# oscar-youngquist/HCR_Genesis_LR_CL

Hardware: AMD Instinct MI355X
Metric: env-steps/sec, Go2 flat 12-DOF, 4096 envs @1/2/4/8 MI355X (higher is better)
Workload: dtype f32

## Files before the change

### hcr_genesis_lr_cl_amd/build.py

```python
import hashlib
import json
import os
import subprocess
import sys
from concurrent.futures import ThreadPoolExecutor

HERE = os.path.dirname(os.path.abspath(__file__))
CSRC = os.path.join(HERE, "csrc")
INC = os.path.join(HERE, "..", "include")
OUT = os.environ.get("LG_BUILD_OUT") or os.path.join(CSRC, "liblgsim.so")
OBJ = os.path.join(CSRC, "obj" if "LG_BUILD_OUT" not in os.environ else "obj_" + os.path.splitext(os.path.basename(OUT))[0])
LLVM_BIN = os.environ.get("LG_LLVM_BIN", "/opt/rocm/lib/llvm/bin")
DPP_PASS = os.environ.get("LG_NO_DPP_PASS", "0") != "1"
PASS_MODE = os.environ.get("LG_DPP_PASS_MODE", "default")
if PASS_MODE not in ("default", "strict"):
    raise ValueError(f"LG_DPP_PASS_MODE={PASS_MODE!r}: expected 'default' or 'strict'")
N_GROUPS = 22
QUAD_GROUPS = list(range(0, 9)) + list(range(17, 22))
COMMON = ["lg_shared.h", "lg_math.h", "lg_lane_ints.h", os.path.join(INC, "lgsim.h")]
EXTRA_FLAGS = os.environ.get("LG_HIPCC_FLAGS", "-fno-slp-vectorize -mllvm -amdgpu-sched-strategy=iterative-ilp").split()
SIDECAR = os.path.splitext(OUT)[0] + ".build.json"
FALLBACK_FLAGS = [["-fno-slp-vectorize", "-mllvm", "-amdgpu-sched-strategy=max-ilp"], ["-fno-slp-vectorize"]]


def units():
    u = [("lg_host", "lg_host.hip", [], COMMON + ["lg_dpp_kat.h"]), ("lg_rollout", "lg_rollout.hip", [], [os.path.join(INC, "lgrollout.h")]),
         ("lg_sensor", "lg_sensor.hip", [], [os.path.join(INC, "lgsensor.h")]),
         ("lg_policy", "lg_policy.hip", [], ["lg_math.h", os.path.join(INC, "lgpolicy.h")]),
         ("lg_ppo", "lg_ppo.hip", [], [os.path.join(INC, "lgppo.h")]),
         ("lg_optim", "lg_optim.hip", [], [os.path.join(INC, "lgoptim.h")]),
         ("lg_train", "lg_train.hip", [], [os.path.join(INC, "lgtrain.h"), os.path.join(INC, "lgpolicy.h"), "lg_train_tiles.h", "lg_train_pass.h"]),
         ("lg_train_ee", "lg_train_ee.hip", [], [os.path.join(INC, "lgtrainee.h"), os.path.join(INC, "lgtrain.h"), os.path.join(INC, "lgpolicy.h"),
                                                 "lg_train_tiles.h", "lg_train_pass.h"]),
         ("lg_train_ts", "lg_train_ts.hip", [], [os.path.join(INC, "lgtraints.h"), os.path.join(INC, "lgtrain.h"), os.path.join(INC, "lgpolicy.h"),
                                                 "lg_train_tiles.h", "lg_train_pass.h"]),
         ("lg_train_dwaq", "lg_train_dwaq.hip", [], [os.path.join(INC, "lgtraindwaq.h"), os.path.join(INC, "lgtrain.h"), os.path.join(INC, "lgpolicy.h"),
                                                     "lg_train_tiles.h", "lg_train_pass.h"]),
         ("lg_train_cts", "lg_train_cts.hip", [], [os.path.join(INC, "lgtraincts.h"), os.path.join(INC, "lgtraints.h"), os.path.join(INC, "lgtrain.h"),
                                                   os.path.join(INC, "lgpolicy.h"), "lg_train_tiles.h", "lg_train_pass.h"]),
         ("lg_train_rnn", "lg_train_rnn.hip", [], [os.path.join(INC, "lgtrainrnn.h"), os.path.join(INC, "lgtrain.h"), os.path.join(INC, "lgpolicy.h"),
                                                   "lg_train_tiles.h", "lg_train_pass.h"]),
         ("lg_train_tcn", "lg_train_tcn.hip", [], [os.path.join(INC, "lgtraintcn.h"), os.path.join(INC, "lgtrain.h"), os.path.join(INC, "lgpolicy.h"),
                                                   "lg_train_tiles.h", "lg_train_pass.h"])]
    for g in range(N_GROUPS):
        deps = COMMON + ["lg_kernel.h"] + (["lg_quad.h"] if g in QUAD_GROUPS else []) + ([os.path.join(HERE, "dpp_hazard_pass.py")] if DPP_PASS else [])
        u.append((f"lg_inst_{g}", "lg_inst.hip", [f"-DLG_GROUP={g}"], deps))
    return u


def _path(f):
    return f if os.path.isabs(f) else os.path.join(CSRC, f)


def source_hash():
    h = hashlib.sha256()
    files = sorted(os.path.join(CSRC, f) for f in os.listdir(CSRC) if f.endswith((".hip", ".h")))
    files += sorted(os.path.join(INC, f) for f in os.listdir(INC) if f.endswith(".h"))
    if DPP_PASS:
        files.append(os.path.join(HERE, "dpp_hazard_pass.py"))
    for f in files:
        h.update(os.path.basename(f).encode())
        with open(f, "rb") as fh:
            h.update(fh.read())
    return h.hexdigest()[:16]


def _unit_key(src, defs, deps, flags):
    h = hashlib.sha256(" ".join(flags + defs + (["dpp-pass", PASS_MODE] if DPP_PASS else [])).encode())
    for f in [src] + list(deps):
# ... 156 lines not shown
```

### hcr_genesis_lr_cl_amd/csrc/lg_host.hip

```cpp
#include "lg_shared.h"
#include "lg_dpp_kat.h"
#include <algorithm>
#include <unistd.h>

__global__ __launch_bounds__(256) void obs_compact_kernel(float *buf, int n_rows, int row, int frame, int stack, int from) {
    const int per = (stack - 1) * frame;
    const long long total = (long long)n_rows * per;
    for (long long t = (long long)blockIdx.x * blockDim.x + threadIdx.x; t < total; t += (long long)gridDim.x * blockDim.x) {
        const int e = (int)(t / per), i = (int)(t % per);
        buf[(size_t)e * row + frame + i] = buf[(size_t)e * row + (size_t)(from + 1) * frame + i];
    }
}

static thread_local std::string g_err;
static int fail(const std::string &m) { g_err = m; return 1; }
int lg_fail_msg(const std::string &m) { return fail(m); }
#define HIPCHK(x) do { hipError_t _e = (x); if (_e != hipSuccess) return fail(std::string(#x) + ": " + hipGetErrorString(_e)); } while (0)

struct LgEngine {
    LgModelDesc model; LgSimOptions opts; LgTaskCfg task;
    LgModelDesc *d_model = nullptr; LgSimOptions *d_opts = nullptr; LgTaskCfg *d_task = nullptr; LgHot *d_hot = nullptr;
    float *d_lane = nullptr;
    const int16_t *hf = nullptr;
    LgBuffers bufs; bool bound = false;
// ... 274 lines not shown
        biped_all_ee = LG_KERNEL((lg_launch_quad<2, true, PR, 6, 3>));
    static constexpr LgKernel quad_prof[4] = {LG_KERNEL((lg_launch_quad<4, true, PR, 1, 3>)), LG_KERNEL((lg_launch_quad<4, true, PR, 2, 3>)),
                                              LG_KERNEL((lg_launch_quad<4, true, PR, 3, 3>)), LG_KERNEL((lg_launch_quad<4, true, PR, 4, 3>))};
    static constexpr LgKernel quad_prof_rs[4] = {LG_KERNEL((lg_launch_quad_rs<4, 1, false>)), LG_KERNEL((lg_launch_quad_rs<4, 2, false>)),
                                                 LG_KERNEL((lg_launch_quad_rs<4, 3, false>)), LG_KERNEL((lg_launch_quad_rs<4, 4, false>))};
    static constexpr LgKernel inj[4] = {{launch_inj<4, 1>, "(lg_launch_quad_inj<4, 1>)"}, {launch_inj<4, 2>, "(lg_launch_quad_inj<4, 2>)"},
                                        {launch_inj<4, 3>, "(lg_launch_quad_inj<4, 3>)"}, {launch_inj<4, 4>, "(lg_launch_quad_inj<4, 4>)"}};
    static constexpr LgKernel inj_rs[4] = {{lg_launch_quad_rs<4, 1, true>, "(lg_launch_quad_inj<4, 1>, reward set constant)"}, {lg_launch_quad_rs<4, 2, true>, "(lg_launch_quad_inj<4, 2>, reward set constant)"},
                                           {lg_launch_quad_rs<4, 3, true>, "(lg_launch_quad_inj<4, 3>, reward set constant)"}, {lg_launch_quad_rs<4, 4, true>, "(lg_launch_quad_inj<4, 4>, reward set constant)"}};
    static constexpr LgKernel inj_biped = {launch_inj<2, 6>, "(lg_launch_quad_inj<2, 6>)"};
    static constexpr LgKernel sole_phys[2] = {LG_KERNEL((lg_launch_quad<LEGS, false, 0u, 0, 4>)), LG_KERNEL((lg_launch_quad<LEGS, true, 0u, 0, 4>))};
    static constexpr LgKernel sole_post_reset = LG_KERNEL((lg_launch_env<LEGS, PR, 0, 4, false>)), sole_post_reset_repl = LG_KERNEL((lg_launch_env<LEGS, PR, 0, 4, true>)),
        sole_post = LG_KERNEL((lg_launch_env<LEGS, LG_PHASE_POST, 0, 4, false>));
};

struct LgPlan { struct { LgKernel k; dim3 grid; } l[2]; int n = 0; bool sim = false; };

template <int LEGS, int JPL> static LgPlan plan(const LgEngine *h, uint32_t ph, const int sw[SW_COUNT]) {
    using K = Kernels<LEGS, JPL>;
    constexpr unsigned PR = K::PR;
    LgPlan pl; pl.sim = (ph & LG_PHASE_SIM) != 0;
    const auto add = [&pl](const LgKernel &k, dim3 grid) { pl.l[pl.n].k = k; pl.l[pl.n].grid = grid; pl.n++; };
    const int threads = h->bufs.n_envs * LEGS;
    const dim3 grid((threads + BLOCK - 1) / BLOCK), qgrid((threads * 4 + BLOCK - 1) / BLOCK), rgrid((threads + 15) / 16);
    const bool pre = (ph & LG_PHASE_PRE) != 0, hfb = hf_bound(h);
    const uint32_t rest = ph & PR;
    const bool repl = sw[SW_MDP_REPLICAS] >= 0 ? sw[SW_MDP_REPLICAS] != 0 : (LEGS == 2 && (long long)threads * 4 <= 1024LL * BLOCK);
    const auto mdp = [&](uint32_t m) {
        if (m == PR) add(repl ? K::post_reset_repl : K::post_reset, repl ? rgrid : grid); else add(K::post, grid); };
    const auto rs = [&](int prof) {
        return (unsigned)h->hot.reward_mask == lg_default_reward_mask(prof) && h->hot.o_contact_iters == LG_DEFAULT_CONTACT_ITERS &&
               h->hot.o_contact_w_every == LG_DEFAULT_CONTACT_W_EVERY && lg_rs_constants_hold(prof, h->task, h->bufs) &&
               sw[SW_REWARD_SET_CONST] != 0; };
    const int layout = h->opts.sim_layout ? h->opts.sim_layout : ((h->quad_ok && (long long)threads * 4 <= 2048LL * BLOCK) ? 2 : 1);
    if (layout == 2 && pl.sim) {
        if constexpr (JPL == 4) {
            add(K::sole_phys[pre], qgrid);
            if (rest == PR) add(repl ? K::sole_post_reset_repl : K::sole_post_reset, repl ? rgrid : grid);
            else if (rest == LG_PHASE_POST) add(K::sole_post, grid);
        } else if (LEGS == 4 && pre && rest == LG_PHASE_POST) {
            add(K::quad_pre_sim_post, qgrid);
        } else if (LEGS == 4 && pre && rest == PR) {
            const int prof = task_profile(h, false);
            add(prof == LG_PROF_NONE ? K::quad_all : rs(prof) ? K::quad_prof_rs[prof - 1] : K::quad_prof[prof - 1], qgrid);
        } else if (LEGS == 2 && pre && rest == PR && sw[SW_BIPED_FUSE] != 0) {
            if (hfb && task_profile(h, false) == LG_PROF_TRON1_PF_EE && sw[SW_BIPED_TAIL] != 0) add(K::biped_all_ee, qgrid);
            else add(hfb ? K::biped_all_hf : K::biped_all, qgrid);
// ... 409 lines not shown
```

### hcr_genesis_lr_cl_amd/csrc/lg_inst.hip

```cpp
#ifndef LG_GROUP
#error "compile with -DLG_GROUP=<0..21> (hcr_genesis_lr_cl_amd/build.py)"
#endif
#include "lg_kernel.h"
#if LG_GROUP < 9 || LG_GROUP >= 17
#include "lg_quad.h"

template <int LEGS, bool PRE, unsigned MPH, int PROF, int JPL>
void lg_launch_quad(dim3 grid, hipStream_t st, hipEvent_t e0, hipEvent_t e1, const KParams &p) {
    const dim3 block(quad_block(PROF, MPH));
    if (e0 || e1) hipExtLaunchKernelGGL((quad_sim_kernel<LEGS, PRE, MPH, PROF, JPL>), grid, block, 0, st, e0, e1, 0, p);
    else hipLaunchKernelGGL((quad_sim_kernel<LEGS, PRE, MPH, PROF, JPL>), grid, block, 0, st, p);
}
#define QUAD(...) template void lg_launch_quad<__VA_ARGS__>(dim3, hipStream_t, hipEvent_t, hipEvent_t, const KParams &);
template <int LEGS, int PROF>
void lg_launch_quad_inj(dim3 grid, hipStream_t st, const KParams &p) {
    constexpr unsigned PR = LG_PHASE_POST | LG_PHASE_RESET;
    hipLaunchKernelGGL((quad_sim_kernel<LEGS, true, PR, PROF, 3, true>), grid, dim3(quad_block(PROF, PR)), 0, st, p);
}
#define QUAD_INJ(...) template void lg_launch_quad_inj<__VA_ARGS__>(dim3, hipStream_t, const KParams &);
template <int LEGS, int PROF, bool INJ>
void lg_launch_quad_rs(dim3 grid, hipStream_t st, hipEvent_t e0, hipEvent_t e1, const KParams &p) {
    constexpr unsigned PR = LG_PHASE_POST | LG_PHASE_RESET;
    const dim3 block(quad_block(PROF, PR));
    if (e0 || e1) hipExtLaunchKernelGGL((quad_sim_kernel<LEGS, true, PR, PROF, 3, INJ, true>), grid, block, 0, st, e0, e1, 0, p);
    else hipLaunchKernelGGL((quad_sim_kernel<LEGS, true, PR, PROF, 3, INJ, true>), grid, block, 0, st, p);
}
#define QUAD_RS(...) template void lg_launch_quad_rs<__VA_ARGS__>(dim3, hipStream_t, hipEvent_t, hipEvent_t, const KParams &);
#else
template <int LEGS, unsigned PH, int PROF, int JPL, bool REPL>
void lg_launch_env(dim3 grid, hipStream_t st, hipEvent_t e0, hipEvent_t e1, const KParams &p) {
    if (e0 || e1) hipExtLaunchKernelGGL((env_step_kernel<LEGS, PH, PROF, JPL, REPL>), grid, dim3(BLOCK), 0, st, e0, e1, 0, p);
    else hipLaunchKernelGGL((env_step_kernel<LEGS, PH, PROF, JPL, REPL>), grid, dim3(BLOCK), 0, st, p);
}
#define ENV(...) template void lg_launch_env<__VA_ARGS__>(dim3, hipStream_t, hipEvent_t, hipEvent_t, const KParams &);
#define ENV_PHASES(LEGS, JPL) ENV(LEGS, 2u, 0, JPL, false) ENV(LEGS, 3u, 0, JPL, false) ENV(LEGS, 4u, 0, JPL, false) ENV(LEGS, 5u, 0, JPL, false) \
                              ENV(LEGS, 7u, 0, JPL, false) ENV(LEGS, 8u, 0, JPL, false)
#endif

#if LG_GROUP == 0
QUAD(4, true, 12u, 1, 3) QUAD(4, true, 4u, 0, 3)
#elif LG_GROUP == 1
QUAD(4, true, 12u, 2, 3)
#elif LG_GROUP == 2
QUAD(4, true, 12u, 3, 3)
#elif LG_GROUP == 3
QUAD(4, true, 12u, 4, 3)
#elif LG_GROUP == 4
QUAD(4, true, 12u, 0, 3)
// ... 38 lines not shown
```

### hcr_genesis_lr_cl_amd/csrc/lg_kernel.h

```cpp
#pragma once
#include "lg_shared.h"

static_assert(LG_R_COUNT <= 32, "reward mask is one dword");
static_assert(sizeof(LgHot) <= 256 * 4, "hot block must fit four dwords per lane");
template <typename T> struct HotGet;
template <> struct HotGet<float> { static LG_DEV float get(int v0, int v1, int v2, int v3, int i) {
    const int v = i < 64 ? v0 : (i < 128 ? v1 : (i < 192 ? v2 : v3)); return __int_as_float(__builtin_amdgcn_readlane(v, i & 63)); } };
template <> struct HotGet<int32_t> { static LG_DEV int get(int v0, int v1, int v2, int v3, int i) {
    const int v = i < 64 ? v0 : (i < 128 ? v1 : (i < 192 ? v2 : v3)); return __builtin_amdgcn_readlane(v, i & 63); } };
template <> struct HotGet<unsigned long long> { static LG_DEV unsigned long long get(int v0, int v1, int v2, int v3, int i) {
    return (unsigned long long)(unsigned)HotGet<int32_t>::get(v0, v1, v2, v3, i) | ((unsigned long long)(unsigned)HotGet<int32_t>::get(v0, v1, v2, v3, i + 1) << 32); } };
template <> struct HotGet<long long> { static LG_DEV long long get(int v0, int v1, int v2, int v3, int i) {
    return (long long)HotGet<unsigned long long>::get(v0, v1, v2, v3, i); } };
#define HOT_OFF(f) ((int)(((size_t) & reinterpret_cast<char const volatile &>(((LgHot *)0)->f)) / 4))
template <typename T> struct HotLds;
template <> struct HotLds<float> { static LG_DEV float get(const int *s, int i) { return __int_as_float(s[i]); } };
template <> struct HotLds<int32_t> { static LG_DEV int get(const int *s, int i) { return __builtin_amdgcn_readfirstlane(s[i]); } };
template <> struct HotLds<unsigned long long> { static LG_DEV unsigned long long get(const int *s, int i) {
    return (unsigned long long)(unsigned)HotLds<int32_t>::get(s, i) | ((unsigned long long)(unsigned)HotLds<int32_t>::get(s, i + 1) << 32); } };
template <> struct HotLds<long long> { static LG_DEV long long get(const int *s, int i) { return (long long)HotLds<unsigned long long>::get(s, i); } };
#define HOT_T(f) typename std::remove_cv<typename std::remove_reference<decltype(((LgHot *)0)->f)>::type>::type
#define CR(k) (__int_as_float(sHot[256 + (k)]))
#define PRG_I(which, dw) (__builtin_amdgcn_readfirstlane(sHot[256 + BLOCK + 26 * (which) + (dw)]))
#define PRG_F(which, dw) (__int_as_float(sHot[256 + BLOCK + 26 * (which) + (dw)]))
// ... 2085 lines not shown
    }
    STAMP(10);
    if (live) {
        B.feet_air_time[e * F + foot_slot] = air;
        B.last_contacts[e * F + foot_slot] = (uint8_t)last_contact;
    }
    if (lead) {
        B.commands[4 * e] = cmd0; B.commands[4 * e + 1] = cmd1; B.commands[4 * e + 2] = cmd2; B.commands[4 * e + 3] = cmd3;
        B.episode_length_buf[e] = ep_len;
        B.fail_buf[e] = fail_buf;
        B.reset_buf[e] = reset ? 1 : 0;
        if (DO_RESET && B.obs_dirty) B.obs_dirty[e] = reset ? 1 : 0;
        B.time_out_buf[e] = time_out ? 1 : 0;
        B.rew_buf[e] = total;
        if (DO_POST || (DO_RESET && reset)) {
#pragma unroll
            for (int k = 0; k < LG_R_COUNT; k++)
                if (RON(k)) esum[(size_t)k * N + e] = es[k];
        }
    }
    STAMP(11);
}

LG_DEV int lg_wg() {
    const int b = (int)blockIdx.x, G = (int)gridDim.x, q = G >> 3, r = G & 7, x = b & 7;
    return x * q + (x < r ? x : r) + (b >> 3);
}

template <int LEGS, unsigned PH, int PROF = 0, int JPL = 3, bool REPL = false>
__global__ __launch_bounds__(BLOCK) void env_step_kernel(KParams p) {
    __shared__ __attribute__((aligned(16))) uint4 sMraw[MODEL_STG * BLOCK];
    __shared__ int sHot[256 + 2 * BLOCK];
    static_assert(!REPL || (PH & (LG_PHASE_PRE | LG_PHASE_SIM)) == 0, "replicated launch: MDP phases only");
    const int vtid = REPL ? (int)(lg_wg() * 16 + (threadIdx.x & 15)) : (int)(lg_wg() * BLOCK + threadIdx.x);
    env_step_body<LEGS, PH, false, PROF, JPL, REPL>(p, sMraw, sHot, nullptr, nullptr, vtid, threadIdx.x & 63);
}
```

### hcr_genesis_lr_cl_amd/csrc/lg_quad.h

```cpp
#pragma once

namespace q4 {

constexpr int QUAD_AXES[4] = {0, 1, 1, 1};

LG_DEV float fsqrt(float x) { return __builtin_amdgcn_sqrtf(x); }

constexpr int QP(int a, int b, int c, int d) { return a | (b << 2) | (c << 4) | (d << 6); }
template <int CTRL> LG_DEV float dpp(float v) {
    return __int_as_float(__builtin_amdgcn_update_dpp(0, __float_as_int(v), CTRL, 0xF, 0xF, true));
}
template <int J> LG_DEV float bc(float v) { return dpp<J * 0x55>(v); }
LG_DEV float bcj(float v, int j) { return j == 0 ? bc<0>(v) : (j == 1 ? bc<1>(v) : (j == 2 ? bc<2>(v) : bc<3>(v))); }
LG_DEV float rot1(float v) { return dpp<QP(1, 2, 0, 3)>(v); }
LG_DEV float rot2(float v) { return dpp<QP(2, 0, 1, 3)>(v); }
LG_DEV float sum3(float t) { return t + rot1(t) + rot2(t); }
LG_DEV float sum4(float t) { t += dpp<QP(1, 0, 3, 2)>(t); return t + dpp<QP(2, 3, 0, 1)>(t); }
LG_DEV int xor4i(int x) {
    int t = __builtin_amdgcn_update_dpp(x, x, 0x104, 0xF, 0x5, false);
    return __builtin_amdgcn_update_dpp(t, x, 0x114, 0xF, 0xA, false);
}
LG_DEV float xor4(float v) { return __int_as_float(xor4i(__float_as_int(v))); }
template <int LEGS> LG_DEV float legsum(float v) {
    if (LEGS == 4) { v += dpp<0x124>(v); v += dpp<0x128>(v); }
// ... 274 lines not shown
    if (wl < head) p[wl] = 0.f;
    float4 *q4p = reinterpret_cast<float4 *>(p + head);
    const int n4 = (n - head) >> 2;
    for (int i = wl; i < n4; i += 64) q4p[i] = make_float4(0.f, 0.f, 0.f, 0.f);
    const int done = head + 4 * n4;
    if (wl < n - done) p[done + wl] = 0.f;
}
LG_DEV void blank_histories(unsigned long long rm, int e, float *obs, size_t orow, int n_o, float *priv, size_t prow, int n_p) {
    const int wl = (int)threadIdx.x & 63;
    while (rm) {
        const int bit = __builtin_ctzll(rm);
        rm &= rm - 1;
        const int er = __builtin_amdgcn_readlane(e, bit);
        zero_run(obs + (size_t)er * orow, n_o, wl);
        zero_run(priv + (size_t)er * prow, n_p, wl);
    }
}

}

constexpr int quad_block(int prof, unsigned mph) { return prof == LG_PROF_TRON1_PF_EE && mph == (LG_PHASE_POST | LG_PHASE_RESET) ? 2 * BLOCK : BLOCK; }

template <int LEGS, bool DO_PRE, unsigned MPH, int PROF = 0, int JPL = 3, bool INJ = false, bool RS = false>
__global__ __launch_bounds__(quad_block(PROF, MPH)) void quad_sim_kernel(KParams p) {
    using namespace q4;
    const unsigned tl_ = threadIdx.x & 63u;
    static_assert(JPL == 3 || (JPL == 4 && LEGS == 2 && MPH == 0 && PROF == LG_PROF_NONE), "four-joint legs: biped physics only");
    constexpr bool FLAT = PROF == LG_PROF_GO2_FLAT, PLANE = FLAT || PROF == LG_PROF_GO2_WTW;
    constexpr bool QTAIL = (PLANE || PROF == LG_PROF_GO2_EE || PROF == LG_PROF_GO2_PROGRAM) && MPH == (LG_PHASE_POST | LG_PHASE_RESET);
    constexpr bool WQ = PROF == LG_PROF_GO2_WTW && QTAIL;
    constexpr bool PQ = PROF == LG_PROF_GO2_PROGRAM && QTAIL;
    constexpr bool EQ = (PROF == LG_PROF_GO2_EE || PROF == LG_PROF_GO2_PROGRAM) && QTAIL;
    constexpr bool SQ = WQ || EQ;
    constexpr bool BQ = PROF == LG_PROF_TRON1_PF_EE && MPH == (LG_PHASE_POST | LG_PHASE_RESET);
    static_assert(PROF != LG_PROF_TRON1_PF_EE || (LEGS == 2 && JPL == 3), "tron1_pf_ee is the three-joint biped's tail");
    constexpr bool CTAIL = QTAIL || BQ;
    constexpr bool GTAIL = MPH != 0 && !CTAIL;
    static_assert(!INJ || (DO_PRE && CTAIL), "injected read-backs: the component-layout tails only");
    constexpr unsigned RS_MASK = lg_default_reward_mask(PROF);
    static_assert(!RS || RS_MASK != 0u, "RS: the profile has a default reward set");
    constexpr int A = JPL * LEGS;
    static_assert(sizeof(KParams) <= 64 * 16, "kernel argument block must fit one dwordx4 per lane");
    const uint4 kq = q4::kernarg_lane((int)(sizeof(KParams) + 15) / 16);
    auto kdw = [&](int dw) {
        const unsigned v = (dw & 3) == 0 ? kq.x : ((dw & 3) == 1 ? kq.y : ((dw & 3) == 2 ? kq.z : kq.w));
        return (unsigned)__builtin_amdgcn_readlane((int)v, dw >> 2);
    };
#define GAS __attribute__((address_space(1)))
#define KPTR(T, off) (reinterpret_cast<T>(((unsigned long long)kdw((int)((off) / 4) + 1) << 32) | (unsigned long long)kdw((int)((off) / 4))))
#define KB(T, f) KPTR(T, offsetof(KParams, B) + offsetof(LgBuffers, f))
#define KINT(member) ((int)kdw((int)(offsetof(KParams, member) / 4)))
#define KFLT(member) (__int_as_float((int)kdw((int)(offsetof(KParams, member) / 4))))
    constexpr bool USE_LT = JPL == 3;
    constexpr bool NEED_M = !USE_LT || GTAIL;
    const LgModelDesc GAS *Mg = KPTR(const LgModelDesc GAS *, offsetof(KParams, M));
    __shared__ __attribute__((aligned(16))) uint4 sMraw[NEED_M ? MODEL_STG * BLOCK : 1];
    __shared__ __attribute__((aligned(16))) uint4 sLT[USE_LT ? LG_LT_STG * BLOCK : 1];
    const LgModelDesc *M = reinterpret_cast<const LgModelDesc *>(sMraw);
    const LgSimOptions *__restrict__ O = p.O;
    __shared__ int sHot[256 + 2 * BLOCK];
    int hv0, hv1, hv2, hv3;
    {
        const int GAS *hp = KPTR(const int GAS *, offsetof(KParams, H)) + (tl_ & 63);
        hv0 = hp[0]; hv1 = hp[64]; hv2 = hp[128]; hv3 = hp[192];
    }
    uint4 stg0 = make_uint4(0u, 0u, 0u, 0u), stg1 = stg0, stg2 = stg0, stg3 = stg0, ltg[LG_LT_STG];
    typedef unsigned int u4v __attribute__((ext_vector_type(4)));
    if constexpr (NEED_M) {
        const u4v GAS *src = reinterpret_cast<const u4v GAS *>(Mg);
        const u4v a0 = src[tl_], a1 = src[tl_ + BLOCK], a2 = src[tl_ + 2 * BLOCK], a3 = src[tl_ + 3 * BLOCK];
        stg0 = make_uint4(a0.x, a0.y, a0.z, a0.w); stg1 = make_uint4(a1.x, a1.y, a1.z, a1.w);
        stg2 = make_uint4(a2.x, a2.y, a2.z, a2.w); stg3 = make_uint4(a3.x, a3.y, a3.z, a3.w);
    }
#pragma unroll
    for (int k = 0; k < LG_LT_STG; k++) ltg[k] = make_uint4(0u, 0u, 0u, 0u);
    if constexpr (USE_LT) {
        const u4v GAS *src = KPTR(const u4v GAS *, offsetof(KParams, LT));
#pragma unroll
        for (int k = 0; k < LG_LT_STG; k++) { const u4v a = src[tl_ + k * BLOCK]; ltg[k] = make_uint4(a.x, a.y, a.z, a.w); }
    }
    const LgBuffers &B = p.B;
    __builtin_amdgcn_sched_barrier(0);
    unsigned long long _stamp0 = 0; (void)_stamp0;
    STAMP(0);
    STAMPB(4096);
    constexpr bool DUO = quad_block(PROF, MPH) == 2 * BLOCK;
    const int wg = lg_wg();
    const int role = DUO ? (int)(threadIdx.x >> 6) : 0;
    const int tid = wg * BLOCK + tl_;
    const int N = KINT(B.n_envs);
    const LgLaneInts LI = lg_lane_ints(tid, N, LEGS, JPL, (unsigned)KINT(k.foot_pack));
    Lane L;
    L.c = LI.c; L.is0 = L.c == 0; L.is1 = L.c == 1; L.is2 = L.c == 2; L.is3 = L.c == 3;
    L.d0 = L.is0 ? 1.f : 0.f; L.d1 = L.is1 ? 1.f : 0.f; L.d2 = L.is2 ? 1.f : 0.f;
    const int cj = LI.cj;
    const int cjj = LI.cjj;
    const int leg = LI.leg, e = LI.e;
    const bool alive = LI.alive != 0;
    const bool live = alive && role == 0;
    const bool st = live && !L.is3;
    const bool stj = JPL == 4 ? live : st;
    const bool lead = st && leg == 0;
    const int nL = KINT(k.m_n_links), F = LEGS;
    const int b0 = 1 + JPL * leg, d0 = JPL * leg;
    const int foot_link = LI.foot_link, foot_slot = LI.foot_slot;

    const float GAS *const k_actions = KB(const float GAS *, actions);
    const float GAS *const k_last_actions = KB(const float GAS *, last_actions);
    const float GAS *const k_base_pos = KB(const float GAS *, base_pos);
    const float GAS *const k_base_lin_vel_w = KB(const float GAS *, base_lin_vel_w);
    const float GAS *const k_base_ang_vel_w = KB(const float GAS *, base_ang_vel_w);
    const float GAS *const k_base_quat = KB(const float GAS *, base_quat);
    const float GAS *const k_dof_pos = KB(const float GAS *, dof_pos);
    const float GAS *const k_dof_vel = KB(const float GAS *, dof_vel);
    const float GAS *const k_feet_vel = KB(const float GAS *, feet_vel);
    const float GAS *const k_base_lin_vel = KB(const float GAS *, base_lin_vel);
    const float GAS *const k_base_ang_vel = KB(const float GAS *, base_ang_vel);
    const float GAS *const k_added_base_mass = KB(const float GAS *, added_base_mass);
    const float GAS *const k_base_com_bias = KB(const float GAS *, base_com_bias);
    const float GAS *const k_friction_values = KB(const float GAS *, friction_values);
    const float GAS *const k_kp_scale = KB(const float GAS *, kp_scale);
    const float GAS *const k_kd_scale = KB(const float GAS *, kd_scale);
    const float GAS *const k_joint_armature = KB(const float GAS *, joint_armature);
    const float GAS *const k_joint_friction = KB(const float GAS *, joint_friction);
    const float GAS *const k_joint_damping = KB(const float GAS *, joint_damping);
    const float GAS *const k_env_origins = KB(const float GAS *, env_origins);
    const float GAS *const k_command_ranges = KB(const float GAS *, command_ranges);
    const float GAS *const k_episode_sums = KB(const float GAS *, episode_sums);
    const float GAS *const k_commands = KB(const float GAS *, commands);
    const float GAS *const k_feet_air_time = KB(const float GAS *, feet_air_time);
    const int32_t GAS *const k_episode_length_buf = KB(const int32_t GAS *, episode_length_buf);
    const int64_t GAS *const k_fail_buf = KB(const int64_t GAS *, fail_buf);
    const uint8_t GAS *const k_last_contacts = KB(const uint8_t GAS *, last_contacts);
    const uint8_t GAS *const k_obs_dirty = KB(const uint8_t GAS *, obs_dirty);
    const float GAS *const k_actions_in = KPTR(const float GAS *, offsetof(KParams, actions));
    const LgSimOptions GAS *kO = KPTR(const LgSimOptions GAS *, offsetof(KParams, O));
    const LgTaskCfg GAS *kT = KPTR(const LgTaskCfg GAS *, offsetof(KParams, T));
    const int ja = LI.ja;
    unsigned o_ja = LI.o_ja, o_e = LI.o_e, o_e3 = LI.o_e3, o_q4 = LI.o_q4, o_fs = LI.o_fs, o_ft = LI.o_ft;
    const unsigned o_dj = LI.o_dj;
    constexpr bool MB = MPH != 0 || DO_PRE;
    float act, last_act = 0.f, llast_act = 0.f;
    if (DO_PRE) {
        const float ca = KFLT(k.clip_actions);
        last_act = ldg(k_actions, o_ja); llast_act = ldg(k_last_actions, o_ja);
        act = clampf(ldg(k_actions_in, o_ja), -ca, ca);
    } else {
        act = k_actions_in ? ldg(k_actions_in, o_ja) : ldg(k_actions, o_ja);
    }
    float pos = ldg(k_base_pos, o_e3), vw = ldg(k_base_lin_vel_w, o_e3), ww = ldg(k_base_ang_vel_w, o_e3);
    float quat = ldg(k_base_quat, o_q4);
    float q = ldg(k_dof_pos, o_ja), qd = ldg(k_dof_vel, o_ja);
    const float snap_fv = ldg(k_feet_vel, o_ft);
    const float snap_blv = ldg(k_base_lin_vel, o_e3), snap_bav = ldg(k_base_ang_vel, o_e3);
    const float dr_mass = (MB || k_added_base_mass) ? ldg(k_added_base_mass, o_e) : 0.f;
    const float dr_com = (MB || k_base_com_bias) ? ldg(k_base_com_bias, o_e3) : 0.f;
    const float dr_fric = (MB || k_friction_values) ? ldg(k_friction_values, o_e) : 1.f;
    const float dr_kp = (MB || k_kp_scale) ? ldg(k_kp_scale, o_ja) : 1.f, dr_kd = (MB || k_kd_scale) ? ldg(k_kd_scale, o_ja) : 1.f;
    float gain_p = 0.f, gain_d = 0.f, q0 = 0.f;
    if constexpr (!USE_LT) { gain_p = kO->kp[d0 + cjj]; gain_d = kO->kd[d0 + cjj]; q0 = kO->default_dof_pos[d0 + cjj]; }
    float dr_arm = 0.f, dr_jf = 0.f, dr_jd = 0.f;
    if (!RS && k_joint_armature) { dr_arm = ldg(k_joint_armature, o_e); dr_jf = ldg(k_joint_friction, o_e); dr_jd = ldg(k_joint_damping, o_e); }
    const float origin = (MB || k_env_origins) ? ldg(k_env_origins, o_e3) : 0.f;
    int crv = 0;
    if (MPH != 0) crv = reinterpret_cast<const int GAS *>(k_command_ranges)[min((int)tl_, LG_CMD_RANGE_FLOATS - 1)];
    int prw = 0;
    if ((MPH & LG_PHASE_RESET) != 0 && (PROF == LG_PROF_GO2_PROGRAM || ((PROF == LG_PROF_NONE || PROF == LG_PROF_NONE_HF) && KINT(k.obs_layout) == LG_OBS_PROGRAM))) {
        const int tl = (int)tl_;
        prw = reinterpret_cast<const int GAS *>(tl < 26 ? &kT->priv_prog : &kT->labels_prog)[tl < 26 ? tl : min(tl - 26, 25)];
    }
    constexpr int NST = LG_R_COUNT + 36;
    __shared__ float sStF[GTAIL ? NST * 16 : 1];
    float wsv[GTAIL ? NST : 1];
    static_assert(LG_R_COUNT <= 32, "two episode sums per lane");
    const int ei = LI.ei;
    float m_cmd = 0.f, m_air = 0.f, m_es0 = 0.f, m_es1 = 0.f, m_slo = 0.f, m_shi = 0.f, m_rlo = 0.f, m_rsp = 0.f, m_nq = 0.f, m_nqd = 0.f;
    int m_ep = 0, m_fail = 0, m_lc = 0;
    float b_es[4] = {0.f, 0.f, 0.f, 0.f}, b_nact = 0.f, b_nclk0 = 0.f, b_nclk1 = 0.f, b_sitq = 0.f, b_sitp = 0.f, b_sitr = 0.f, b_th0 = 0.f, b_th1 = 0.f;
    unsigned o_es = LI.o_es;
    if (BQ) {
        static_assert(LG_R_COUNT <= 32, "four episode sums per lane");
#pragma unroll
        for (int k = 0; k < 4; k++) if (ei + 8 * k < LG_R_COUNT) b_es[k] = ldg(k_episode_sums, o_es + 32u * (unsigned)k * (unsigned)N);
        b_nact = ldg(&kT->noise_vec[9 + 2 * A], o_dj);
        b_nclk0 = ldg(&kT->noise_vec[9 + 3 * A], 4u * (unsigned)foot_slot); b_nclk1 = ldg(&kT->noise_vec[9 + 3 * A + LEGS], 4u * (unsigned)foot_slot);
        b_sitq = ldg(&kT->sit_dof_pos[0], o_dj); b_sitp = ldg(&kT->sit_pos[0], 4u * (unsigned)cj); b_sitr = ldg(&kT->sit_quat[0], 4u * (unsigned)L.c);
        b_th0 = kT->theta_table[0][0]; b_th1 = kT->theta_table[0][1];
    }
    if (CTAIL) {
        m_cmd = ldg(k_commands, o_q4);
        m_ep = ldg(k_episode_length_buf, o_e);
        m_fail = (int)ldg(k_fail_buf, 2u * o_e);
        m_air = ldg(k_feet_air_time, o_fs);
        m_lc = (int)ldg(k_last_contacts, o_fs >> 2);
        if (QTAIL) m_es0 = ldg(k_episode_sums, o_es);
        if (QTAIL && ei + 16 < LG_R_COUNT) m_es1 = ldg(k_episode_sums, o_es + 64u * (unsigned)N);
        m_slo = ldg(&kT->soft_dof_lo[0], o_dj); m_shi = ldg(&kT->soft_dof_hi[0], o_dj);
        m_rlo = ldg(&kT->reset_dof_lo[0], o_dj); m_rsp = ldg(&kT->reset_dof_span[0], o_dj);
        m_nq = ldg(&kT->noise_vec[9], o_dj); m_nqd = ldg(&kT->noise_vec[9 + A], o_dj);
    }
    float w_gt = 0.f, w_phi = 0.f, w_gp = 1.f, w_bh = 0.f, w_fc = 0.f, w_pt = 0.f, w_th = 0.f, w_ec = 0.f, w_push = 0.f;
    int w_dirty = 0, w_lvl = 0, w_type = 0;
// ... 24 lines not shown
        int fsL = 0;
#pragma unroll
        for (int k = 0; k < LEGS; k++) fsL += (KINT(k.m_foot_link[k]) < flL) ? 1 : 0;
#pragma unroll
        for (int k = 0; k < LG_R_COUNT; k++) wsv[k] = k_episode_sums[(size_t)k * N + eL];
        int c2 = LG_R_COUNT;
#pragma unroll
        for (int j = 0; j < 3; j++) {
            wsv[c2++] = T->soft_dof_lo[dL + j]; wsv[c2++] = T->soft_dof_hi[dL + j];
            wsv[c2++] = T->reset_dof_lo[dL + j]; wsv[c2++] = T->reset_dof_span[dL + j];
            wsv[c2++] = T->noise_vec[9 + dL + j]; wsv[c2++] = T->noise_vec[9 + A + dL + j]; wsv[c2++] = T->noise_vec[9 + 2 * A + dL + j];
        }
        const bool clk = KINT(k.obs_layout) == LG_OBS_TRON1_EE;
        wsv[c2++] = clk ? T->noise_vec[9 + 3 * A + fsL] : 0.f; wsv[c2++] = clk ? T->noise_vec[9 + 3 * A + LEGS + fsL] : 0.f;
        wsv[c2++] = k_commands[4 * eL]; wsv[c2++] = k_commands[4 * eL + 1]; wsv[c2++] = k_commands[4 * eL + 2]; wsv[c2++] = k_commands[4 * eL + 3];
        wsv[c2++] = __int_as_float(k_episode_length_buf[eL]);
        wsv[c2++] = __int_as_float((int)k_fail_buf[eL]);
        wsv[c2++] = k_feet_air_time[eL * F + fsL];
        wsv[c2++] = __int_as_float((int)k_last_contacts[eL * F + fsL]);
        wsv[c2++] = k_env_origins[3 * eL]; wsv[c2++] = k_env_origins[3 * eL + 1]; wsv[c2++] = k_env_origins[3 * eL + 2];
        wsv[c2++] = __int_as_float(((MPH & LG_PHASE_RESET) && k_obs_dirty) ? (int)k_obs_dirty[eL] : 0);
    }

    asm volatile("" ::: "memory");
    sHot[tl_] = hv0; sHot[tl_ + 64] = hv1; sHot[tl_ + 128] = hv2; sHot[tl_ + 192] = hv3;
    if (MPH != 0) {
        sHot[tl_ + 256] = crv;
        sHot[tl_ + 256 + BLOCK] = prw;
        if (!CTAIL && tl_ < 16) {
            const unsigned rm = p.k.reward_mask;
            const bool leadL = (wg * 16 + tl_) % LEGS == 0;
#pragma unroll
            for (int k = 0; k < LG_R_COUNT; k++) sStF[k * 16 + tl_] = (leadL && ((rm >> k) & 1u)) ? wsv[k] : 0.f;
#pragma unroll
            for (int k = LG_R_COUNT; k < NST - 1; k++) sStF[k * 16 + tl_] = wsv[k];
        }
    }
    if constexpr (NEED_M) { sMraw[tl_] = stg0; sMraw[tl_ + BLOCK] = stg1; sMraw[tl_ + 2 * BLOCK] = stg2; sMraw[tl_ + 3 * BLOCK] = stg3; }
    if constexpr (USE_LT) {
#pragma unroll
        for (int k = 0; k < LG_LT_STG; k++) sLT[tl_ + k * BLOCK] = ltg[k];
    }
    if (DUO) __builtin_amdgcn_s_waitcnt(0x0F70);
    __syncthreads();
    STAMP(23);

// ... 1921 lines not shown
```

### hcr_genesis_lr_cl_amd/csrc/lg_shared.h

```cpp
#pragma once
#include <hip/hip_runtime.h>
#include <initializer_list>
#include <stdint.h>
#include <stdio.h>
#include <string.h>
#include <string>
#include <type_traits>
#include "../../include/lgsim.h"
#include "lg_math.h"
#include "lg_lane_ints.h"
#include <vector>
#include <hip/hip_ext.h>

#define LG_ABI_VERSION 3
#define BLOCK 64
#define MODEL_STG 4
static_assert(sizeof(LgModelDesc) <= MODEL_STG * BLOCK * 16, "model table does not fit the staging image");

struct LgHot {
    int32_t obs_layout;
    int32_t num_obs;
    int32_t num_priv_obs;
    int32_t obs_frame;
    int32_t priv_frame;
    int32_t obs_stack;
    int32_t priv_stack;
    int32_t obs_slack;
// ... 291 lines not shown
    }
}

struct KParams {
    const LgModelDesc *M;
    const LgSimOptions *O;
    const LgTaskCfg *T;
    const LgHot *H;
    const float *LT;
    const int16_t *hf;
    LgBuffers B;
    const float *actions;
    long long counter;
    int jrot_identity;
    struct { int m_n_links, m_foot_link[4], obs_layout, o_n_height_points; unsigned reward_mask; float clip_actions;
             int cat_enable;
             int joint_axis[4];
             unsigned foot_pack;
    } k;
    int obs_win;
    int obs_set;
};

enum : int { LG_PROF_NONE = 0, LG_PROF_GO2_FLAT = 1, LG_PROF_GO2_WTW = 2, LG_PROF_GO2_EE = 3, LG_PROF_GO2_PROGRAM = 4,
             LG_PROF_NONE_HF = 5,
             LG_PROF_TRON1_PF_EE = 6 };

template <int LEGS, bool PRE, unsigned MPH, int PROF, int JPL>
void lg_launch_quad(dim3 grid, hipStream_t st, hipEvent_t e0, hipEvent_t e1, const KParams &p);
template <int LEGS, unsigned PH, int PROF, int JPL, bool REPL>
void lg_launch_env(dim3 grid, hipStream_t st, hipEvent_t e0, hipEvent_t e1, const KParams &p);
template <int LEGS, int PROF>
void lg_launch_quad_inj(dim3 grid, hipStream_t st, const KParams &p);
constexpr unsigned lg_default_reward_mask(int prof) {
    return prof == LG_PROF_GO2_FLAT ? 0x26a2296fu : prof == LG_PROF_GO2_WTW ? 0x7f2c0967u : (prof == LG_PROF_GO2_EE || prof == LG_PROF_GO2_PROGRAM) ? 0x242a6567u : 0u;
}
constexpr int LG_DEFAULT_CONTACT_ITERS = 2, LG_DEFAULT_CONTACT_W_EVERY = 1;
struct LgProfFlags { int heading_command, only_positive_rewards, dr_friction_on, dr_mass_on, dr_com_on, dr_pd_on, custom_origins; };
constexpr LgProfFlags lg_default_flags(int prof) {
    return LgProfFlags{1, 1, 1, 1, 1, prof == LG_PROF_GO2_FLAT ? 0 : 1, (prof == LG_PROF_GO2_EE || prof == LG_PROF_GO2_PROGRAM) ? 1 : 0};
}
inline bool lg_rs_constants_hold(int prof, const LgTaskCfg &t, const LgBuffers &b) {
    const LgProfFlags f = lg_default_flags(prof);
    const bool ok = (t.heading_command != 0) == (f.heading_command != 0) &&
              (t.only_positive_rewards != 0) == (f.only_positive_rewards != 0) && (t.dr_friction_on != 0) == (f.dr_friction_on != 0) &&
              (t.dr_mass_on != 0) == (f.dr_mass_on != 0) && (t.dr_com_on != 0) == (f.dr_com_on != 0) && (t.dr_pd_on != 0) == (f.dr_pd_on != 0) &&
// ... 14 lines not shown
```

Before: 165.7 million.

## Preload a kernel-argument head into SGPRs and hoist early loads in quad kernel

Adds a 14-dword argument head (LT, H, n_envs, foot_pack and four action/base pointers) ahead of KParams. The quad kernel groups are compiled with amdgpu kernarg preloading, so these values arrive in SGPRs instead of waiting on the per-lane kernarg read and readlane extraction. The first global loads (actions, last actions, base position) are hoisted before the remaining kernarg decoding, and the workgroup swizzle uses a grid size computed from n_envs rather than gridDim. A host-side grid check aborts on a mismatched grid. Debug timestamp probes are added behind LG_DBG_STAMPS. This trades a larger argument block and duplicated fields for lower startup latency in a short, launch-bound kernel.

Result: no change. 164.7 million (-0.6%).

```diff
diff --git a/hcr_genesis_lr_cl_amd/build.py b/hcr_genesis_lr_cl_amd/build.py
--- a/hcr_genesis_lr_cl_amd/build.py
+++ b/hcr_genesis_lr_cl_amd/build.py
@@ -17,6 +17,7 @@
     raise ValueError(f"LG_DPP_PASS_MODE={PASS_MODE!r}: expected 'default' or 'strict'")
 N_GROUPS = 22
 QUAD_GROUPS = list(range(0, 9)) + list(range(17, 22))
+PRELOAD_FLAGS = ["-mllvm", "-amdgpu-kernarg-preload-count=8"]
 COMMON = ["lg_shared.h", "lg_math.h", "lg_lane_ints.h", os.path.join(INC, "lgsim.h")]
 EXTRA_FLAGS = os.environ.get("LG_HIPCC_FLAGS", "-fno-slp-vectorize -mllvm -amdgpu-sched-strategy=iterative-ilp").split()
 SIDECAR = os.path.splitext(OUT)[0] + ".build.json"
@@ -44,7 +45,7 @@
                                                    "lg_train_tiles.h", "lg_train_pass.h"])]
     for g in range(N_GROUPS):
         deps = COMMON + ["lg_kernel.h"] + (["lg_quad.h"] if g in QUAD_GROUPS else []) + ([os.path.join(HERE, "dpp_hazard_pass.py")] if DPP_PASS else [])
-        u.append((f"lg_inst_{g}", "lg_inst.hip", [f"-DLG_GROUP={g}"], deps))
+        u.append((f"lg_inst_{g}", "lg_inst.hip", [f"-DLG_GROUP={g}"] + (PRELOAD_FLAGS if g in QUAD_GROUPS else []), deps))
     return u
 
 
diff --git a/hcr_genesis_lr_cl_amd/csrc/lg_host.hip b/hcr_genesis_lr_cl_amd/csrc/lg_host.hip
--- a/hcr_genesis_lr_cl_amd/csrc/lg_host.hip
+++ b/hcr_genesis_lr_cl_amd/csrc/lg_host.hip
@@ -320,7 +320,7 @@
     LgPlan pl; pl.sim = (ph & LG_PHASE_SIM) != 0;
     const auto add = [&pl](const LgKernel &k, dim3 grid) { pl.l[pl.n].k = k; pl.l[pl.n].grid = grid; pl.n++; };
     const int threads = h->bufs.n_envs * LEGS;
-    const dim3 grid((threads + BLOCK - 1) / BLOCK), qgrid((threads * 4 + BLOCK - 1) / BLOCK), rgrid((threads + 15) / 16);
+    const dim3 grid((threads + BLOCK - 1) / BLOCK), qgrid(lg_quad_grid(h->bufs.n_envs, LEGS)), rgrid((threads + 15) / 16);
     const bool pre = (ph & LG_PHASE_PRE) != 0, hfb = hf_bound(h);
     const uint32_t rest = ph & PR;
     const bool repl = sw[SW_MDP_REPLICAS] >= 0 ? sw[SW_MDP_REPLICAS] != 0 : (LEGS == 2 && (long long)threads * 4 <= 1024LL * BLOCK);
diff --git a/hcr_genesis_lr_cl_amd/csrc/lg_inst.hip b/hcr_genesis_lr_cl_amd/csrc/lg_inst.hip
--- a/hcr_genesis_lr_cl_amd/csrc/lg_inst.hip
+++ b/hcr_genesis_lr_cl_amd/csrc/lg_inst.hip
@@ -8,22 +8,28 @@
 template <int LEGS, bool PRE, unsigned MPH, int PROF, int JPL>
 void lg_launch_quad(dim3 grid, hipStream_t st, hipEvent_t e0, hipEvent_t e1, const KParams &p) {
     const dim3 block(quad_block(PROF, MPH));
-    if (e0 || e1) hipExtLaunchKernelGGL((quad_sim_kernel<LEGS, PRE, MPH, PROF, JPL>), grid, block, 0, st, e0, e1, 0, p);
-    else hipLaunchKernelGGL((quad_sim_kernel<LEGS, PRE, MPH, PROF, JPL>), grid, block, 0, st, p);
+    lg_quad_grid_check(grid, p, LEGS);
+    const KHead hd = lg_khead(p);
+    if (e0 || e1) hipExtLaunchKernelGGL((quad_sim_kernel<LEGS, PRE, MPH, PROF, JPL>), grid, block, 0, st, e0, e1, 0, LG_KHEAD_ARGS(hd), p);
+    else hipLaunchKernelGGL((quad_sim_kernel<LEGS, PRE, MPH, PROF, JPL>), grid, block, 0, st, LG_KHEAD_ARGS(hd), p);
 }
 #define QUAD(...) template void lg_launch_quad<__VA_ARGS__>(dim3, hipStream_t, hipEvent_t, hipEvent_t, const KParams &);
 template <int LEGS, int PROF>
 void lg_launch_quad_inj(dim3 grid, hipStream_t st, const KParams &p) {
     constexpr unsigned PR = LG_PHASE_POST | LG_PHASE_RESET;
-    hipLaunchKernelGGL((quad_sim_kernel<LEGS, true, PR, PROF, 3, true>), grid, dim3(quad_block(PROF, PR)), 0, st, p);
+    lg_quad_grid_check(grid, p, LEGS);
+    const KHead hd = lg_khead(p);
+    hipLaunchKernelGGL((quad_sim_kernel<LEGS, true, PR, PROF, 3, true>), grid, dim3(quad_block(PROF, PR)), 0, st, LG_KHEAD_ARGS(hd), p);
 }
 #define QUAD_INJ(...) template void lg_launch_quad_inj<__VA_ARGS__>(dim3, hipStream_t, const KParams &);
 template <int LEGS, int PROF, bool INJ>
 void lg_launch_quad_rs(dim3 grid, hipStream_t st, hipEvent_t e0, hipEvent_t e1, const KParams &p) {
     constexpr unsigned PR = LG_PHASE_POST | LG_PHASE_RESET;
     const dim3 block(quad_block(PROF, PR));
-    if (e0 || e1) hipExtLaunchKernelGGL((quad_sim_kernel<LEGS, true, PR, PROF, 3, INJ, true>), grid, block, 0, st, e0, e1, 0, p);
-    else hipLaunchKernelGGL((quad_sim_kernel<LEGS, true, PR, PROF, 3, INJ, true>), grid, block, 0, st, p);
+    lg_quad_grid_check(grid, p, LEGS);
+    const KHead hd = lg_khead(p);
+    if (e0 || e1) hipExtLaunchKernelGGL((quad_sim_kernel<LEGS, true, PR, PROF, 3, INJ, true>), grid, block, 0, st, e0, e1, 0, LG_KHEAD_ARGS(hd), p);
+    else hipLaunchKernelGGL((quad_sim_kernel<LEGS, true, PR, PROF, 3, INJ, true>), grid, block, 0, st, LG_KHEAD_ARGS(hd), p);
 }
 #define QUAD_RS(...) template void lg_launch_quad_rs<__VA_ARGS__>(dim3, hipStream_t, hipEvent_t, hipEvent_t, const KParams &);
 #else
diff --git a/hcr_genesis_lr_cl_amd/csrc/lg_kernel.h b/hcr_genesis_lr_cl_amd/csrc/lg_kernel.h
--- a/hcr_genesis_lr_cl_amd/csrc/lg_kernel.h
+++ b/hcr_genesis_lr_cl_amd/csrc/lg_kernel.h
@@ -2131,10 +2131,11 @@
     STAMP(11);
 }
 
-LG_DEV int lg_wg() {
-    const int b = (int)blockIdx.x, G = (int)gridDim.x, q = G >> 3, r = G & 7, x = b & 7;
+LG_DEV int lg_wg(const int G) {
+    const int b = (int)blockIdx.x, q = G >> 3, r = G & 7, x = b & 7;
     return x * q + (x < r ? x : r) + (b >> 3);
 }
+LG_DEV int lg_wg() { return lg_wg((int)gridDim.x); }
 
 template <int LEGS, unsigned PH, int PROF = 0, int JPL = 3, bool REPL = false>
 __global__ __launch_bounds__(BLOCK) void env_step_kernel(KParams p) {
diff --git a/hcr_genesis_lr_cl_amd/csrc/lg_quad.h b/hcr_genesis_lr_cl_amd/csrc/lg_quad.h
--- a/hcr_genesis_lr_cl_amd/csrc/lg_quad.h
+++ b/hcr_genesis_lr_cl_amd/csrc/lg_quad.h
@@ -320,8 +320,16 @@
 constexpr int quad_block(int prof, unsigned mph) { return prof == LG_PROF_TRON1_PF_EE && mph == (LG_PHASE_POST | LG_PHASE_RESET) ? 2 * BLOCK : BLOCK; }
 
 template <int LEGS, bool DO_PRE, unsigned MPH, int PROF = 0, int JPL = 3, bool INJ = false, bool RS = false>
-__global__ __launch_bounds__(quad_block(PROF, MPH)) void quad_sim_kernel(KParams p) {
+__global__ __launch_bounds__(quad_block(PROF, MPH)) void quad_sim_kernel(LG_KHEAD_PARAMS, KParams p) {
     using namespace q4;
+#ifdef LG_DBG_STAMPS
+    unsigned long long _t_in;
+    asm volatile("s_memtime %0\n\ts_waitcnt lgkmcnt(0)" : "=s"(_t_in) :: "memory");
+#define STAMP_IN(i, dep) do { unsigned long long _t; asm volatile("s_memtime %0\n\ts_waitcnt lgkmcnt(0)" : "=s"(_t) : "s"(dep) : "memory"); \
+    if (blockIdx.x == 0 && threadIdx.x == 0) p.B.episode_done_sums[i] = (float)(long long)(_t - _t_in); } while (0)
+#else
+#define STAMP_IN(i, dep) do { } while (0)
+#endif
     const unsigned tl_ = threadIdx.x & 63u;
     static_assert(JPL == 3 || (JPL == 4 && LEGS == 2 && MPH == 0 && PROF == LG_PROF_NONE), "four-joint legs: biped physics only");
     constexpr bool FLAT = PROF == LG_PROF_GO2_FLAT, PLANE = FLAT || PROF == LG_PROF_GO2_WTW;
@@ -338,12 +346,14 @@
     constexpr unsigned RS_MASK = lg_default_reward_mask(PROF);
     static_assert(!RS || RS_MASK != 0u, "RS: the profile has a default reward set");
     constexpr int A = JPL * LEGS;
-    static_assert(sizeof(KParams) <= 64 * 16, "kernel argument block must fit one dwordx4 per lane");
-    const uint4 kq = q4::kernarg_lane((int)(sizeof(KParams) + 15) / 16);
-    auto kdw = [&](int dw) {
+    static_assert(sizeof(KHead) + sizeof(KParams) <= 64 * 16, "kernel argument head and block must fit one dwordx4 per lane");
+    const uint4 kq = q4::kernarg_lane((int)(sizeof(KHead) + sizeof(KParams) + 15) / 16);
+    auto kdw = [&](int dw_) {
+        const int dw = dw_ + LG_KHEAD_DWORDS;
         const unsigned v = (dw & 3) == 0 ? kq.x : ((dw & 3) == 1 ? kq.y : ((dw & 3) == 2 ? kq.z : kq.w));
         return (unsigned)__builtin_amdgcn_readlane((int)v, dw >> 2);
     };
+#define HPTR(T, h) (reinterpret_cast<T>((unsigned long long)(h)))
 #define GAS __attribute__((address_space(1)))
 #define KPTR(T, off) (reinterpret_cast<T>(((unsigned long long)kdw((int)((off) / 4) + 1) << 32) | (unsigned long long)kdw((int)((off) / 4))))
 #define KB(T, f) KPTR(T, offsetof(KParams, B) + offsetof(LgBuffers, f))
@@ -359,7 +369,7 @@
     __shared__ int sHot[256 + 2 * BLOCK];
     int hv0, hv1, hv2, hv3;
     {
-        const int GAS *hp = KPTR(const int GAS *, offsetof(KParams, H)) + (tl_ & 63);
+        const int GAS *hp = HPTR(const int GAS *, h_H) + (tl_ & 63);
         hv0 = hp[0]; hv1 = hp[64]; hv2 = hp[128]; hv3 = hp[192];
     }
     uint4 stg0 = make_uint4(0u, 0u, 0u, 0u), stg1 = stg0, stg2 = stg0, stg3 = stg0, ltg[LG_LT_STG];
@@ -373,7 +383,7 @@
 #pragma unroll
     for (int k = 0; k < LG_LT_STG; k++) ltg[k] = make_uint4(0u, 0u, 0u, 0u);
     if constexpr (USE_LT) {
-        const u4v GAS *src = KPTR(const u4v GAS *, offsetof(KParams, LT));
+        const u4v GAS *src = HPTR(const u4v GAS *, h_LT);
 #pragma unroll
         for (int k = 0; k < LG_LT_STG; k++) { const u4v a = src[tl_ + k * BLOCK]; ltg[k] = make_uint4(a.x, a.y, a.z, a.w); }
     }
@@ -381,13 +391,14 @@
     __builtin_amdgcn_sched_barrier(0);
     unsigned long long _stamp0 = 0; (void)_stamp0;
     STAMP(0);
+    STAMP_IN(28, 0);
     STAMPB(4096);
     constexpr bool DUO = quad_block(PROF, MPH) == 2 * BLOCK;
-    const int wg = lg_wg();
+    const int wg = lg_wg((int)lg_quad_grid(h_n_envs, LEGS));
     const int role = DUO ? (int)(threadIdx.x >> 6) : 0;
     const int tid = wg * BLOCK + tl_;
-    const int N = KINT(B.n_envs);
-    const LgLaneInts LI = lg_lane_ints(tid, N, LEGS, JPL, (unsigned)KINT(k.foot_pack));
+    const int N = h_n_envs;
+    const LgLaneInts LI = lg_lane_ints(tid, N, LEGS, JPL, h_foot_pack);
     Lane L;
     L.c = LI.c; L.is0 = L.c == 0; L.is1 = L.c == 1; L.is2 = L.c == 2; L.is3 = L.c == 3;
     L.d0 = L.is0 ? 1.f : 0.f; L.d1 = L.is1 ? 1.f : 0.f; L.d2 = L.is2 ? 1.f : 0.f;
@@ -399,13 +410,30 @@
     const bool st = live && !L.is3;
     const bool stj = JPL == 4 ? live : st;
     const bool lead = st && leg == 0;
-    const int nL = KINT(k.m_n_links), F = LEGS;
+    constexpr int F = LEGS;
     const int b0 = 1 + JPL * leg, d0 = JPL * leg;
     const int foot_link = LI.foot_link, foot_slot = LI.foot_slot;
-
-    const float GAS *const k_actions = KB(const float GAS *, actions);
-    const float GAS *const k_last_actions = KB(const float GAS *, last_actions);
-    const float GAS *const k_base_pos = KB(const float GAS *, base_pos);
+    const int ja = LI.ja;
+    unsigned o_ja = LI.o_ja, o_e = LI.o_e, o_e3 = LI.o_e3, o_q4 = LI.o_q4, o_fs = LI.o_fs, o_ft = LI.o_ft;
+    const unsigned o_dj = LI.o_dj;
+    unsigned o_es = LI.o_es;
+
+    __builtin_amdgcn_sched_barrier(0);
+    const float GAS *const k_actions_in = HPTR(const float GAS *, h_actions_in);
+    const float GAS *const k_actions = HPTR(const float GAS *, h_actions);
+    const float GAS *const k_last_actions = HPTR(const float GAS *, h_last_actions);
+    const float GAS *const k_base_pos = HPTR(const float GAS *, h_base_pos);
+    float act, last_act = 0.f, llast_act = 0.f;
+    if (DO_PRE) {
+        last_act = ldg(k_actions, o_ja); llast_act = ldg(k_last_actions, o_ja);
+        act = ldg(k_actions_in, o_ja);
+    } else {
+        act = k_actions_in ? ldg(k_actions_in, o_ja) : ldg(k_actions, o_ja);
+    }
+    float pos = ldg(k_base_pos, o_e3);
+    __builtin_amdgcn_sched_barrier(0);
+    const int nL = KINT(k.m_n_links);
+    STAMP_IN(29, nL);
     const float GAS *const k_base_lin_vel_w = KB(const float GAS *, base_lin_vel_w);
     const float GAS *const k_base_ang_vel_w = KB(const float GAS *, base_ang_vel_w);
     const float GAS *const k_base_quat = KB(const float GAS *, base_quat);
@@ -431,22 +459,14 @@
     const int64_t GAS *const k_fail_buf = KB(const int64_t GAS *, fail_buf);
     const uint8_t GAS *const k_last_contacts = KB(const uint8_t GAS *, last_contacts);
     const uint8_t GAS *const k_obs_dirty = KB(const uint8_t GAS *, obs_dirty);
-    const float GAS *const k_actions_in = KPTR(const float GAS *, offsetof(KParams, actions));
     const LgSimOptions GAS *kO = KPTR(const LgSimOptions GAS *, offsetof(KParams, O));
     const LgTaskCfg GAS *kT = KPTR(const LgTaskCfg GAS *, offsetof(KParams, T));
-    const int ja = LI.ja;
-    unsigned o_ja = LI.o_ja, o_e = LI.o_e, o_e3 = LI.o_e3, o_q4 = LI.o_q4, o_fs = LI.o_fs, o_ft = LI.o_ft;
-    const unsigned o_dj = LI.o_dj;
     constexpr bool MB = MPH != 0 || DO_PRE;
-    float act, last_act = 0.f, llast_act = 0.f;
     if (DO_PRE) {
         const float ca = KFLT(k.clip_actions);
-        last_act = ldg(k_actions, o_ja); llast_act = ldg(k_last_actions, o_ja);
-        act = clampf(ldg(k_actions_in, o_ja), -ca, ca);
-    } else {
-        act = k_actions_in ? ldg(k_actions_in, o_ja) : ldg(k_actions, o_ja);
-    }
-    float pos = ldg(k_base_pos, o_e3), vw = ldg(k_base_lin_vel_w, o_e3), ww = ldg(k_base_ang_vel_w, o_e3);
+        act = clampf(act, -ca, ca);
+    }
+    float vw = ldg(k_base_lin_vel_w, o_e3), ww = ldg(k_base_ang_vel_w, o_e3);
     float quat = ldg(k_base_quat, o_q4);
     float q = ldg(k_dof_pos, o_ja), qd = ldg(k_dof_vel, o_ja);
     const float snap_fv = ldg(k_feet_vel, o_ft);
@@ -475,7 +495,6 @@
     float m_cmd = 0.f, m_air = 0.f, m_es0 = 0.f, m_es1 = 0.f, m_slo = 0.f, m_shi = 0.f, m_rlo = 0.f, m_rsp = 0.f, m_nq = 0.f, m_nqd = 0.f;
     int m_ep = 0, m_fail = 0, m_lc = 0;
     float b_es[4] = {0.f, 0.f, 0.f, 0.f}, b_nact = 0.f, b_nclk0 = 0.f, b_nclk1 = 0.f, b_sitq = 0.f, b_sitp = 0.f, b_sitr = 0.f, b_th0 = 0.f, b_th1 = 0.f;
-    unsigned o_es = LI.o_es;
     if (BQ) {
         static_assert(LG_R_COUNT <= 32, "four episode sums per lane");
 #pragma unroll
@@ -546,6 +565,7 @@
         wsv[c2++] = __int_as_float(((MPH & LG_PHASE_RESET) && k_obs_dirty) ? (int)k_obs_dirty[eL] : 0);
     }
 
+    STAMP_IN(30, 0);
     asm volatile("" ::: "memory");
     sHot[tl_] = hv0; sHot[tl_ + 64] = hv1; sHot[tl_ + 128] = hv2; sHot[tl_ + 192] = hv3;
     if (MPH != 0) {
diff --git a/hcr_genesis_lr_cl_amd/csrc/lg_shared.h b/hcr_genesis_lr_cl_amd/csrc/lg_shared.h
--- a/hcr_genesis_lr_cl_amd/csrc/lg_shared.h
+++ b/hcr_genesis_lr_cl_amd/csrc/lg_shared.h
@@ -3,6 +3,7 @@
 #include <initializer_list>
 #include <stdint.h>
 #include <stdio.h>
+#include <stdlib.h>
 #include <string.h>
 #include <string>
 #include <type_traits>
@@ -340,6 +341,36 @@
     int obs_set;
 };
 
+struct KHead {
+    const float *LT;
+    const LgHot *H;
+    int n_envs;
+    unsigned foot_pack;
+    const float *actions_in;
+    const float *actions;
+    const float *last_actions;
+    const float *base_pos;
+};
+#define LG_KHEAD_DWORDS 14
+#define LG_KHEAD_PARAMS const float *h_LT, const LgHot *h_H, int h_n_envs, unsigned h_foot_pack, const float *h_actions_in, const float *h_actions, \
+                        const float *h_last_actions, const float *h_base_pos
+#define LG_KHEAD_ARGS(hd) (hd).LT, (hd).H, (hd).n_envs, (hd).foot_pack, (hd).actions_in, (hd).actions, (hd).last_actions, (hd).base_pos
+static_assert(sizeof(KHead) == 4 * LG_KHEAD_DWORDS && offsetof(KHead, LT) == 0 && offsetof(KHead, H) == 8 && offsetof(KHead, n_envs) == 16 &&
+              offsetof(KHead, foot_pack) == 20 && offsetof(KHead, actions_in) == 24 && offsetof(KHead, actions) == 32 &&
+              offsetof(KHead, last_actions) == 40 && offsetof(KHead, base_pos) == 48, "the head is the kernel-argument segment's first 14 dwords, member by member");
+static_assert(sizeof(KHead) % alignof(KParams) == 0, "KParams follows the head without padding (lg_quad.h kdw)");
+static_assert(sizeof(KHead) % 8 == 0 && offsetof(KParams, B) % 8 == 0 && offsetof(KParams, actions) % 8 == 0, "a pointer's two dwords stay in one 16-byte lane (lg_quad.h KPTR)");
+__host__ __device__ constexpr unsigned lg_quad_grid(int n_envs, int legs) { return ((unsigned)n_envs * (unsigned)legs * 4u + BLOCK - 1u) / BLOCK; }
+inline void lg_quad_grid_check(dim3 grid, const KParams &p, int legs) {
+    if (grid.x != lg_quad_grid(p.B.n_envs, legs) || grid.y != 1u || grid.z != 1u) {
+        fprintf(stderr, "quad_sim_kernel: grid %u x %u x %u for %d envs of %d legs (lg_quad_grid: %u)\n", grid.x, grid.y, grid.z, p.B.n_envs, legs, lg_quad_grid(p.B.n_envs, legs));
+        abort();
+    }
+}
+inline KHead lg_khead(const KParams &p) {
+    return KHead{p.LT, p.H, p.B.n_envs, p.k.foot_pack, p.actions, p.B.actions, p.B.last_actions, p.B.base_pos};
+}
+
 enum : int { LG_PROF_NONE = 0, LG_PROF_GO2_FLAT = 1, LG_PROF_GO2_WTW = 2, LG_PROF_GO2_EE = 3, LG_PROF_GO2_PROGRAM = 4,
              LG_PROF_NONE_HF = 5,
              LG_PROF_TRON1_PF_EE = 6 };
```
